# pastas/metran

Hardware: AMD Instinct MI355X
Metric: Kalman filter+smoother steps/sec (batched DFMs) (higher is better)
Workload: dtype f64

## Files before the change

include/metran_hip.h:

```cpp
#ifndef METRAN_HIP_H
#define METRAN_HIP_H

#include <stddef.h>
#include <stdint.h>

#ifdef __cplusplus
extern "C" {
#endif

#define MK_API __attribute__((visibility("default")))
#define MK_ABI_VERSION 7

typedef enum mk_status {
    MK_OK = 0,
    MK_ERR_INVALID = -1,
    MK_ERR_SHAPE = -2,
    MK_ERR_HIP = -3,
    MK_ERR_NO_DEVICE = -4,
    MK_ERR_ALLOC = -5
} mk_status;

#define MK_FLAG_NONPOSITIVE_F 1u
#define MK_FLAG_NOT_SPD 2u
#define MK_FLAG_RANK_DEFICIENT 4u
// ... 151 lines not shown
                           int64_t ndraws, int antithetic, int64_t T, int64_t ncomp, int raw, double *d_out);

MK_API int64_t mk_path_functional_count(void);
MK_API int mk_path_functionals(mk_context *ctx, const mk_problem *prob , int64_t ndraws,
                               int what , int time_major, const double *d_paths, int64_t W,
                               const int64_t *d_windows , const double *d_thresholds ,
                               double *d_functionals );
MK_API int64_t mk_ensemble_max_draws(void);
MK_API int mk_ensemble_summary(mk_context *ctx, int64_t S, int64_t cells, const double *d_values , int64_t nprobs,
                               const double *probs , double *d_summary );

typedef struct mk_weights_request {
    int64_t n_targets;
    int what;
    const int64_t *d_targets;
    double *d_weights;
    double *d_intercept;
} mk_weights_request;
MK_API int64_t mk_weights_work_stride(int64_t N, int64_t K);
MK_API int mk_observation_weights(mk_context *ctx, const mk_problem *prob, double *d_work, int time_major,
                                  const mk_weights_request *req, uint32_t *d_status);

MK_API int mk_smooth(mk_context *ctx, const mk_problem *prob, const mk_outputs *out);

MK_API int mk_filter_smooth(mk_context *ctx, const mk_problem *prob, const mk_outputs *out);

MK_API int mk_simulate(mk_context *ctx, int64_t B, int64_t RZ, int64_t T, int64_t N, int64_t n,
                       const double *d_Z, const double *d_means ,
                       const double *d_covs , double *d_sim_means ,
                       double *d_sim_vars );

MK_API int mk_decompose(mk_context *ctx, int64_t B, int64_t RZ, int64_t T, int64_t N, int64_t n,
                        const double *d_Z, const double *d_means ,
                        double *d_sdf , double *d_cdf );

MK_API int mk_sum(mk_context *ctx, int64_t count, const double *d_values, double *d_result );

MK_API int mk_comm_set_library(const char *path);
MK_API int mk_comm_unique_id(void *id128 );
MK_API int mk_comm_init_rank(mk_context *ctx, int nranks, int rank, const void *id128);
MK_API int mk_set_communicator(mk_context *ctx, void *nccl_comm);
MK_API int mk_comm_destroy(mk_context *ctx);
MK_API int mk_allreduce_sum(mk_context *ctx, double *d_buf, int64_t count);

MK_API int mk_standardize(mk_context *ctx, int64_t R, int64_t T, int64_t N, int time_major,
                          const double *d_in, double *d_out, double *d_mean, double *d_std);
// ... 29 lines not shown
```

metran_amd/_lib.py:

```python
import ctypes
import os
from ctypes import POINTER, Structure, c_char_p, c_double, c_float, c_int, c_int64, c_size_t, c_uint32, c_uint64, c_void_p

__all__ = ["MetranHipError", "lib", "library_path", "Problem", "Outputs", "ForecastRequest", "WeightsRequest", "check", "API"]

_HERE = os.path.dirname(os.path.abspath(__file__))
_LIBNAME = "libmetran_hip.so"


class MetranHipError(Exception):
    """Raised for every failure of the HIP library (the reference raises bare ``Exception``
    with a logged message, e.g. /root/reference/metran/kalmanfilter.py:733-745)."""


c_dp = POINTER(c_double)
c_i64p = POINTER(c_int64)
c_u32p = POINTER(c_uint32)


class Problem(Structure):

    _fields_ = [
        ("n_instances", c_int64),
        ("n_records", c_int64),
# ... 73 lines not shown
    "mk_sync": (c_int, [c_void_p]),
    "mk_observations_changed": (c_int, [c_void_p]),
    "mk_shape_supported": (c_int, [c_int64, c_int64]),
    "mk_shape_specialised": (c_int, [c_int64, c_int64]),
    "mk_generic_max_states": (c_int64, []),
    "mk_register_shape_module": (c_int, [c_char_p]),
    "mk_record_stride": (c_int64, [c_int64]),
    "mk_record_stride_sym": (c_int64, [c_int64]),
    "mk_tape_stride": (c_int64, [c_int64, c_int64]),
    "mk_tape_supported": (c_int, [c_int64, c_int64]),
    "mk_state_tape_stride": (c_int64, [c_int64, c_int64]),
    "mk_supported_shapes": (c_int, [c_i64p, c_int]),
    "mk_malloc": (c_int, [c_void_p, c_size_t, POINTER(c_void_p)]),
    "mk_free": (c_int, [c_void_p, c_void_p]),
    "mk_memcpy_h2d": (c_int, [c_void_p, c_void_p, c_void_p, c_size_t]),
    "mk_memcpy_d2h": (c_int, [c_void_p, c_void_p, c_void_p, c_size_t]),
    "mk_memset": (c_int, [c_void_p, c_void_p, c_int, c_size_t]),
    "mk_params_from_alpha": (c_int, [c_void_p, c_int64, c_int64, c_int64, c_int64, c_void_p, c_void_p, c_double,
                                     c_void_p, c_void_p]),
    "mk_filter": (c_int, [c_void_p, POINTER(Problem), POINTER(Outputs)]),
    "mk_loglik": (c_int, [c_void_p, POINTER(Problem), c_void_p]),
    "mk_smooth": (c_int, [c_void_p, POINTER(Problem), POINTER(Outputs)]),
    "mk_filter_smooth": (c_int, [c_void_p, POINTER(Problem), POINTER(Outputs)]),
    "mk_smooth_dense": (c_int, [c_void_p, c_int64, c_int64, c_int64, c_void_p, c_void_p, c_void_p, c_void_p, c_void_p, c_void_p,
                                c_void_p, c_void_p]),
    "mk_simulate": (c_int, [c_void_p, c_int64, c_int64, c_int64, c_int64, c_int64, c_void_p, c_void_p, c_void_p,
                            c_void_p, c_void_p]),
    "mk_decompose": (c_int, [c_void_p, c_int64, c_int64, c_int64, c_int64, c_int64, c_void_p, c_void_p, c_void_p,
                             c_void_p]),
    "mk_sum": (c_int, [c_void_p, c_int64, c_void_p, c_void_p]),
    "mk_comm_set_library": (c_int, [c_char_p]),
    "mk_comm_unique_id": (c_int, [c_void_p]),
    "mk_comm_init_rank": (c_int, [c_void_p, c_int, c_int, c_void_p]),
    "mk_set_communicator": (c_int, [c_void_p, c_void_p]),
    "mk_comm_destroy": (c_int, [c_void_p]),
    "mk_allreduce_sum": (c_int, [c_void_p, c_void_p, c_int64]),
    "mk_loglik_grad": (c_int, [c_void_p, POINTER(Problem), c_void_p, c_int, c_void_p, c_void_p, c_void_p, c_void_p, c_void_p]),
    "mk_loglik_grad_phases": (c_int, [c_void_p, POINTER(Problem), c_void_p, c_int, c_void_p, c_void_p, c_void_p, c_void_p, c_void_p,
                                      c_int]),
    "mk_adjoint_update_stride": (c_int64, [c_int64, c_int64]),
    "mk_set_adjoint_updates": (c_int, [c_void_p, c_void_p, c_int64]),
    "mk_lbfgs_direction": (c_int, [c_void_p, c_int64, c_int64, c_int64, c_void_p, c_void_p, c_void_p, c_void_p, c_void_p, c_void_p, c_void_p,
                                   c_void_p, c_void_p, c_double, c_void_p, c_void_p, c_void_p, c_void_p, c_void_p, POINTER(c_int)]),
    "mk_lbfgs_trial": (c_int, [c_void_p, c_int64, c_int64, c_void_p, c_void_p, c_void_p, c_void_p, c_void_p, c_void_p, c_void_p, c_void_p]),
    "mk_lbfgs_armijo": (c_int, [c_void_p, c_int64, c_int64, c_void_p, c_void_p, c_void_p, c_void_p, c_void_p, c_void_p, c_void_p, c_void_p,
                                c_void_p, c_void_p, c_int64, c_void_p, POINTER(c_int), POINTER(c_int)]),
# ... 82 lines not shown
```

metran_amd/csrc/mk_capi.hip:

```cpp
#include <hip/hip_runtime.h>

#include <cmath>
#include <cstdarg>
#include <cstdio>
#include <cstring>
#include <dlfcn.h>
#include <mutex>
#include <vector>
#include <new>

#include "draw_kernels.h"
#include "ensemble_kernels.h"
#include "forecast_kernels.h"
#include "innov_kernels.h"
#include "mk_generic.h"
#include "mk_internal.h"
#include "mk_lbfgs.h"
#include "weights_kernels.h"

struct mk_context {
    int device;
    hipStream_t stream;
    int timing;
    hipEvent_t ev[4];
    bool have_filter_time, have_smooth_time;
    std::vector<hipEvent_t> ev_pool;
    std::vector<std::pair<hipEvent_t, hipEvent_t>> ev_pending[2];
    int *tlist;
    long tlist_cap;
    const double *tlist_obs;
    long tlist_T, tlist_N, tlist_ostep;
    unsigned char *lr_take;
    long lr_cap;
    int *lr_any_dev;
    const double *lr_obs;
    long lr_R, lr_T, lr_N, lr_bs;
    int lr_any;
    int variant[MK_VARIANT_COUNT];
    double *gws;
    size_t gws_cap;
    int *lb_counters;
    double *adj_upd;
    size_t adj_upd_cap;
    double *cur_upd;
    void *comm;
    bool comm_owned;
};

static thread_local char g_err[512] = "";

static int fail(int code, const char *fmt, ...)
{
    va_list ap;
    va_start(ap, fmt);
    vsnprintf(g_err, sizeof(g_err), fmt, ap);
// ... 91 lines not shown
            hipError_t e = hipStreamSynchronize(ctx->stream);
            if (e != hipSuccess) return e;
            e = hipFree(ctx->gws);
            if (e != hipSuccess) return e;
        }
        ctx->gws = nullptr;
        ctx->gws_cap = 0;
        const hipError_t e = hipMalloc((void **)&ctx->gws, need * sizeof(double));
        if (e != hipSuccess) return e;
        ctx->gws_cap = need;
    }
    *ws = ctx->gws;
    return hipSuccess;
}
hipError_t dispatch_smoother(mk_context *ctx, int N, int K, const mk::SmootherArgs &a, hipStream_t s)
{
    const bool proj = a.sim_means || a.sim_vars || a.tape != 0;
    const bool force_generic = ctx->variant[MK_VARIANT_KERNEL_FAMILY] == 1;
    if (!force_generic) {
        if (const mk::ShapeOps *o = find_ops(N, K)) return o->smoother(a, s);
        if (!proj)
            if (const mk::ShapeOps *o = find_ops(N, K, true)) {
                mk::SmootherArgs b = a;
                b.obs = nullptr;
                return o->smoother(b, s);
            }
    }
    if (generic_shape(N, K)) {
        mk::GenericSmootherArgs g;
        g.a = a;
        g.N = N;
        g.K = K;
        g.Xp = g.Pp = nullptr;
        const hipError_t e = generic_workspace(ctx, a.B, N + K, &g.ws);
        if (e != hipSuccess) return e;
        return mk::launch_smoother_generic(g, s);
    }
    return hipErrorInvalidValue;
}
}

template <class Args>
static void fill_model(Args &a, const mk_problem *p)
{
    a.B = p->n_instances;
    a.R = p->n_records;
    a.T = p->T;
// ... 96 lines not shown
{
    if (!out) return fail(MK_ERR_INVALID, "null ctx out-pointer");
    *out = nullptr;
    int c = 0;
    if (hipGetDeviceCount(&c) != hipSuccess || c <= 0)
        return fail(MK_ERR_NO_DEVICE, "no HIP device visible (libmetran_hip needs an MI355X / gfx950)");
    if (device < 0 || device >= c) return fail(MK_ERR_INVALID, "device %d out of range [0,%d)", device, c);
    MK_HIP(hipSetDevice(device));
    hipDeviceProp_t prop;
    MK_HIP(hipGetDeviceProperties(&prop, device));
    if (strncmp(prop.gcnArchName, "gfx950", 6) != 0)
        return fail(MK_ERR_NO_DEVICE, "device %d is %s; this library is built for gfx950 only", device,
                    prop.gcnArchName);
    mk_context *ctx = new (std::nothrow) mk_context();
    if (!ctx) return fail(MK_ERR_ALLOC, "out of host memory");
    ctx->device = device;
    ctx->stream = nullptr;
    ctx->timing = 0;
    ctx->have_filter_time = ctx->have_smooth_time = false;
    ctx->tlist = nullptr;
    ctx->tlist_cap = 0;
    ctx->tlist_obs = nullptr;
    ctx->tlist_T = ctx->tlist_N = ctx->tlist_ostep = 0;
    ctx->lr_take = nullptr;
    ctx->lr_cap = 0;
    ctx->lr_any_dev = nullptr;
    ctx->lr_obs = nullptr;
    ctx->lr_R = ctx->lr_T = ctx->lr_N = ctx->lr_bs = 0;
    ctx->lr_any = 0;
    ctx->gws = nullptr;
    ctx->gws_cap = 0;
    ctx->lb_counters = nullptr;
    ctx->comm = nullptr;
    ctx->comm_owned = false;
    ctx->adj_upd = ctx->cur_upd = nullptr;
    ctx->adj_upd_cap = 0;
    for (int &v : ctx->variant) v = 0;
    for (auto &e : ctx->ev) {
        if (hipEventCreate(&e) != hipSuccess) {
            delete ctx;
            return fail(MK_ERR_HIP, "hipEventCreate failed");
        }
    }
    *out = ctx;
    return MK_OK;
}

// ... 122 lines not shown
        return fail(MK_ERR_INVALID, "mk_allreduce_sum: this context has no communicator -- call mk_comm_init_rank (every rank, with "
                                    "the id of mk_comm_unique_id) or mk_set_communicator first; there is no single-rank shortcut");
    if (!d_buf || count <= 0) return fail(MK_ERR_INVALID, "mk_allreduce_sum: bad argument");
    MK_HIP(hipSetDevice(ctx->device));
    const RcclApi *api = rccl_api();
    if (!api) return fail(MK_ERR_HIP, "mk_allreduce_sum: %s", g_rccl.why);
    MK_RCCL(api, api->AllReduce(d_buf, d_buf, (size_t)count, kNcclFloat64, kNcclSum, ctx->comm, ctx->stream));
    return MK_OK;
}

MK_API int mk_destroy(mk_context *ctx)
{
    if (!ctx) return MK_OK;
    (void)hipSetDevice(ctx->device);
    for (auto &e : ctx->ev) (void)hipEventDestroy(e);
    for (auto &e : ctx->ev_pool) (void)hipEventDestroy(e);
    for (auto &v : ctx->ev_pending)
        for (auto &pr : v) {
            (void)hipEventDestroy(pr.first);
            (void)hipEventDestroy(pr.second);
        }
    if (ctx->tlist) (void)hipFree(ctx->tlist);
    if (ctx->gws) (void)hipFree(ctx->gws);
    if (ctx->lr_take) (void)hipFree(ctx->lr_take);
    if (ctx->lr_any_dev) (void)hipFree(ctx->lr_any_dev);
    if (ctx->lb_counters) (void)hipFree(ctx->lb_counters);
    (void)mk_comm_destroy(ctx);
    delete ctx;
    return MK_OK;
}

MK_API int mk_set_stream(mk_context *ctx, void *s)
{
    MK_CTX(ctx);
    if (ctx->stream != (hipStream_t)s) ctx->tlist_obs = ctx->lr_obs = nullptr;
    ctx->stream = (hipStream_t)s;
    return MK_OK;
}

MK_API int mk_set_kernel_variant(mk_context *ctx, int which, int value)
{
    MK_CTX(ctx);
    if (which < 0 || which >= MK_VARIANT_COUNT) return fail(MK_ERR_INVALID, "mk_set_kernel_variant: unknown selector %d", which);
    if (value < 0 || value > ((which == MK_VARIANT_SINGLE_RECORD || which == MK_VARIANT_KERNEL_FAMILY || which == MK_VARIANT_TAPE_FILTER) ? 1 : 2))
        return fail(MK_ERR_INVALID, "mk_set_kernel_variant: value must be 0 or 1 (0, 1 or 2 for the smoother selectors and the wide filter)");
    ctx->variant[which] = value;
    return MK_OK;
// ... 257 lines not shown
    a.detfs = o->d_detfs;
    a.sigmacount = (long long *)o->d_sigmacount;
    a.F = o->d_F;
    a.Pf = o->d_Pf;
    a.Xp = o->d_Xp;
    a.Pp = o->d_Pp;
    a.status = o->d_status;
    if ((a.sym || a.tape) && (!specialised(p->N, p->K) || ctx->variant[MK_VARIANT_KERNEL_FAMILY] == 1))
        return fail(MK_ERR_SHAPE, "packed-symmetric records and the tape exist for specialised shapes only (N=%lld, K=%lld runs the size-generic "
                                  "kernels: mk_shape_specialised)", (long long)p->N, (long long)p->K);
    MK_HIP(timing_start(ctx, 0));
    {
        const hipError_t e = dispatch_filter((int)p->N, (int)p->K, a, ctx->stream, ctx->variant[MK_VARIANT_KERNEL_FAMILY] == 1);
        if (e == hipErrorNotSupported)
            return fail(MK_ERR_SHAPE, "a model of N=%lld series and K=%lld factors is not served on this device in this mode (the size-generic "
                                      "filter keeps the %lld x %lld covariance in LDS: %zu bytes)", (long long)p->N, (long long)p->K,
                        (long long)(p->N + p->K), (long long)(p->N + p->K), mk::generic_filter_lds_bytes((int)p->N, (int)p->K));
        MK_HIP(e);
    }
    MK_HIP(timing_stop(ctx, 0));
    return MK_OK;
}

static hipError_t full_records(mk_context *ctx, const mk_problem *p, const unsigned char **take)
{
    *take = nullptr;
    const long bs = p->obs_time_major ? 1 : p->T;
    if (!(ctx->lr_obs == p->d_obs && ctx->lr_R == p->n_records && ctx->lr_T == p->T && ctx->lr_N == p->N && ctx->lr_bs == bs)) {
        hipStreamCaptureStatus cap = hipStreamCaptureStatusNone;
        if (hipStreamIsCapturing(ctx->stream, &cap) != hipSuccess) (void)hipGetLastError();
        if (cap != hipStreamCaptureStatusNone) return hipSuccess;
        ctx->lr_obs = nullptr;
        if (ctx->lr_cap < p->n_records) {
            if (ctx->lr_take) {
                hipError_t e = hipStreamSynchronize(ctx->stream);
                if (e != hipSuccess) return e;
                (void)hipFree(ctx->lr_take);
                ctx->lr_take = nullptr;
                ctx->lr_cap = 0;
            }
            hipError_t e = hipMalloc((void **)&ctx->lr_take, (size_t)p->n_records);
            if (e != hipSuccess) return e;
            ctx->lr_cap = p->n_records;
        }
        if (!ctx->lr_any_dev) {
            hipError_t e = hipMalloc((void **)&ctx->lr_any_dev, sizeof(int));
            if (e != hipSuccess) return e;
        }
        hipError_t e = hipMemsetAsync(ctx->lr_any_dev, 0, sizeof(int), ctx->stream);
        if (e != hipSuccess) return e;
        e = mk::launch_full_records(p->n_records, p->T, (int)p->N, bs, p->obs_time_major ? p->n_records : 1, p->d_obs, ctx->lr_take,
                                    ctx->lr_any_dev, ctx->stream);
        if (e != hipSuccess) return e;
        e = hipMemcpyAsync(&ctx->lr_any, ctx->lr_any_dev, sizeof(int), hipMemcpyDeviceToHost, ctx->stream);
        if (e != hipSuccess) return e;
        e = hipStreamSynchronize(ctx->stream);
        if (e != hipSuccess) return e;
        ctx->lr_obs = p->d_obs;
        ctx->lr_R = p->n_records;
        ctx->lr_T = p->T;
        ctx->lr_N = p->N;
        ctx->lr_bs = bs;
    }
    if (ctx->lr_any) *take = ctx->lr_take;
    return hipSuccess;
}

static int do_smooth(mk_context *ctx, const mk_problem *p, const mk_outputs *o, bool clear_status)
{
    const int tape = tape_outputs(p, o);
    if (tape < 0) return tape;
    if (!o->d_F || (!o->d_Pf && !tape))
        return fail(MK_ERR_INVALID, "the smoother reads d_F and d_Pf (filtered moments); both must be non-NULL");
    if (tape == 1 && !(o->d_sim_means || o->d_sim_vars))
        return fail(MK_ERR_INVALID, "MK_OUT_TAPE: nothing to write, give d_sim_means / d_sim_vars");
    mk::SmootherArgs a;
    a.tape = tape;
    a.obsvar = tape ? p->d_obsvar : nullptr;
    a.variant = (ctx->variant[MK_VARIANT_SMOOTHER16] == 1 ? 1 : 0) | (ctx->variant[MK_VARIANT_WIDE_SMOOTHER] == 1 ? 2 : 0) |
                (ctx->variant[MK_VARIANT_WIDE_SMOOTHER] == 2 ? 4 : 0);
    a.rs = 0;
    a.sym = 0;
    a.state_means = a.state_vars = nullptr;
    const bool sym = (o->flags & MK_OUT_PACKED_SYM) != 0, var = (o->flags & MK_OUT_VAR_ONLY) != 0;
    if (tape) {
        a.rs = o->record_stride;
    } else if (o->record_stride) {
        const int64_t n = p->N + p->K;
        const int64_t want = sym ? mk::record_stride_sym((int)n) : mk::record_stride((int)n);
        if (o->record_stride != want)
            return fail(MK_ERR_INVALID, "record_stride must be %s(n) = %lld doubles", sym ? "mk_record_stride_sym" : "mk_record_stride",
                        (long long)want);
        const bool proj = o->d_sim_means || o->d_sim_vars;
        if (o->d_Pf != o->d_F + n) return fail(MK_ERR_INVALID, "record layout needs d_Pf = d_F + n");
        if (var) {
            if (!o->d_S || !o->d_Ps || proj)
                return fail(MK_ERR_INVALID, "MK_OUT_VAR_ONLY needs d_S [B,T,n] (means) and d_Ps [B,T,n] (variances), no projection outputs");
        } else {
            if ((o->d_S || o->d_Ps) && !(o->d_S && o->d_Ps == o->d_S + n))
                return fail(MK_ERR_INVALID, "record layout needs a smoothed record array d_S with d_Ps = d_S + n");
            if (!o->d_S && !proj)
                return fail(MK_ERR_INVALID, "nothing to write: give d_S/d_Ps records or d_sim_means/d_sim_vars");
        }
        if (proj && !p->d_loadings) return fail(MK_ERR_INVALID, "the projection outputs need d_loadings");
        a.rs = o->record_stride;
        a.sym = sym ? 1 : 0;
    } else if (o->d_sim_means || o->d_sim_vars || sym || var) {
        return fail(MK_ERR_INVALID, "d_sim_means / d_sim_vars, MK_OUT_PACKED_SYM and MK_OUT_VAR_ONLY need the record layout "
                                    "(record_stride = mk_record_stride[_sym](n))");
    }
    a.obs = nullptr;
    a.lr_take = nullptr;
    a.obs_bs = a.obs_ts = 0;
    if (p->d_obs && p->d_loadings && !p->d_obsvar && !tape && ctx->variant[MK_VARIANT_SMOOTHER16] != 2 &&
        (double)p->n_records * (double)p->T * (double)p->N * sizeof(double) < 4294967296.0) {
        const bool served = !sym && !var && o->record_stride && !(o->d_sim_means || o->d_sim_vars) && p->N + p->K <= 10 &&
                            ctx->variant[MK_VARIANT_SMOOTHER16] == 0 && ctx->variant[MK_VARIANT_KERNEL_FAMILY] == 0;
        if (served) MK_HIP(full_records(ctx, p, &a.lr_take));
        if (a.lr_take) {
            a.obs = p->d_obs;
            a.obs_bs = p->obs_time_major ? 1 : p->T;
            a.obs_ts = p->obs_time_major ? p->n_records : 1;
        }
    }
    a.R = p->n_records;
    a.loadings = p->d_loadings;
    fill_scaling(a, p);
    a.sim_means = o->d_sim_means;
    a.sim_vars = o->d_sim_vars;
    a.B = p->n_instances;
    a.T = p->T;
    fill_layout(a, (int)o->time_major, p->n_instances, p->T);
    a.phi = p->d_phi;
    a.q = p->d_q;
    a.F = o->d_F;
    a.Pf = o->d_Pf;
    if (tape == 2 && !p->d_loadings) return fail(MK_ERR_INVALID, "the state tape needs d_loadings");
    a.S = var ? nullptr : o->d_S;
    a.Ps = var ? nullptr : o->d_Ps;
    if (var) {
        a.state_means = o->d_S;
        a.state_vars = o->d_Ps;
    }
    a.status = o->d_status;
    MK_HIP(timing_start(ctx, 1));
    if ((sym || tape) && (!specialised(p->N, p->K) || ctx->variant[MK_VARIANT_KERNEL_FAMILY] == 1))
// ... 979 lines not shown
```

metran_amd/csrc/mk_ingest.hip:

```cpp
#include <hip/hip_runtime.h>

#include "mk_internal.h"

namespace mk {

__global__ void __launch_bounds__(256)
standardize_kernel(long R, long T, int N, long bs, long ts, const double *in, double *out, double *mean,
                   double *stdev)
{
    __shared__ double s_sum[256];
    __shared__ long s_cnt[256];
    __shared__ double s_mean[64], s_std[64];
    const long r = blockIdx.x;
    const int RP = 256 / N, tid = threadIdx.x;
    const int j = tid % N, row0 = tid / N;
    const bool active = row0 < RP;
    const double *src = in + r * bs * N;

    double acc = 0.0;
    long cnt = 0;
    if (active)
        for (long t = row0; t < T; t += RP) {
            const double y = src[t * ts * N + j];
            if (y == y) {
// ... 78 lines not shown
hipError_t launch_standardize(long R, long T, int N, int time_major, const double *in, double *out, double *mean,
                              double *stdev, hipStream_t s)
{
    const long bs = time_major ? 1 : T, ts = time_major ? R : 1;
    hipLaunchKernelGGL(standardize_kernel, dim3((unsigned)R), dim3(256), 0, s, R, T, N, bs, ts, in, out, mean, stdev);
    return hipGetLastError();
}

hipError_t launch_mask(long count, const double *obs, const unsigned char *mask, double *out, hipStream_t s)
{
    hipLaunchKernelGGL(mask_kernel, dim3((unsigned)((count + 255) / 256)), dim3(256), 0, s, count, obs, mask, out);
    return hipGetLastError();
}

hipError_t launch_pack(long RT, int N, const double *obs, double *observations, double *indices, long *count,
                       hipStream_t s)
{
    hipLaunchKernelGGL(pack_kernel, dim3((unsigned)((RT + 255) / 256)), dim3(256), 0, s, RT, N, obs, observations,
                       indices, count);
    return hipGetLastError();
}

__global__ void __launch_bounds__(256)
full_records_kernel(long T, int N, long obs_bs, long obs_ts, const double *obs, unsigned char *take, int *any)
{
    __shared__ unsigned s_cnt;
    if (threadIdx.x == 0) s_cnt = 0u;
    __syncthreads();
    const double *src = obs + (long)blockIdx.x * obs_bs * N;
    unsigned cnt = 0;
    for (long t = threadIdx.x; t < T; t += 256) {
        bool full = true;
        for (int j = 0; j < N; ++j) full = full && isfinite(src[t * obs_ts * N + j]);
        cnt += full ? 1u : 0u;
    }
    atomicAdd(&s_cnt, cnt);
    __syncthreads();
    if (threadIdx.x == 0) {
        const bool ok = 8ull * s_cnt >= 7ull * (unsigned long long)T;
        take[blockIdx.x] = ok ? 1 : 0;
        if (ok) atomicOr(any, 1);
    }
}

hipError_t launch_full_records(long R, long T, int N, long obs_bs, long obs_ts, const double *obs, unsigned char *take, int *any,
                               hipStream_t s)
{
    hipLaunchKernelGGL(full_records_kernel, dim3((unsigned)R), dim3(256), 0, s, T, N, obs_bs, obs_ts, obs, take, any);
    return hipGetLastError();
}

}
```

metran_amd/csrc/mk_internal.h:

```cpp
#pragma once
#include <hip/hip_runtime.h>

#include "metran_hip.h"

#ifndef MK_SHAPES
#define MK_SHAPES(X) \
    X(8, 2)          \
    X(5, 1)          \
    X(2, 1)          \
    X(3, 1)          \
    X(4, 1)          \
    X(6, 2)          \
    X(14, 3)         \
    X(32, 4)
#endif

namespace mk {

constexpr int wave_smoother_max_n = 51;

constexpr int tape_side_c(int K) { return K + 4; }
constexpr int tape_xs_c(int N, int K) { return N + tape_side_c(K); }
constexpr int tape_ss_c(int N, int K) { return tape_xs_c(N, K); }
constexpr int tape_so_c(int N, int K) { return N; }
// ... 23 lines not shown

#ifdef MK_TUNE
#define MK_TUNE_SKIP(args, bit) (((MK_TUNE) & (bit)) != 0)
#else
#define MK_TUNE_SKIP(args, bit) false
#endif

struct SmootherArgs {
    long B, T;
    long bs, ts;
    long rs;
    long sym;
    double *state_means, *state_vars;
    long R;
    const double *loadings, *scale, *offset;
    double *sim_means, *sim_vars;
    const double *phi, *q;
    const double *F, *Pf;
    double *S, *Ps;
    unsigned *status;
    long variant;
    long tape;
    const double *obsvar;
    const double *obs;
    long obs_bs, obs_ts;
    const unsigned char *lr_take;
};

struct AdjointArgs {
    long B, R, T, warmup;
    long bs, ts, rs;
    long obs_bs, obs_ts;
    const double *obs, *phi, *q, *loadings, *obsvar, *x0, *P0;
    const double *F;
    const long long *sigmacount;
    double *gphi, *gq;
    const double *upd;
    long us;
    double *loo_means, *loo_vars;
    const double *scale, *offset;
    double *dist_r, *dist_n;
};

enum class AdjointMode { Grad, Loo, Dist };

struct SparseArgs {
    long B, T, warmup;
    long ostep;
    const double *obs;
    const double *phi, *q, *loadings, *obsvar, *x0, *P0;
// ... 25 lines not shown
    hipError_t (*disturb)(const AdjointArgs &, hipStream_t);
};
const ShapeOps *shape_ops(int *count);
constexpr int module_abi()
{
    return (int)(sizeof(FilterArgs) * 1000 + sizeof(SmootherArgs) + sizeof(AdjointArgs) + sizeof(SparseArgs) + sizeof(ShapeOps));
}
hipError_t launch_alpha_grad(long B, long R, int N, int K, const double *alpha, const double *loadings, double dt,
                             const double *gphi, const double *gq, double *galpha, hipStream_t s);
int record_stride(int n);
int record_stride_sym(int n);
hipError_t launch_params(long B, long R, int N, int K, const double *alpha, const double *loadings, double dt,
                         double *phi, double *q, hipStream_t s);
hipError_t launch_simulate(long B, long RZ, long T, int N, int n, const double *Z, const double *means,
                           const double *covs, double *sm, double *sv, hipStream_t s);
hipError_t launch_decompose(long B, long RZ, long T, int N, int n, const double *Z, const double *means,
                            double *sdf, double *cdf, hipStream_t s);
hipError_t launch_sum(long count, const double *v, double *out, hipStream_t s);
hipError_t launch_standardize(long R, long T, int N, int time_major, const double *in, double *out, double *mean,
                              double *stdev, hipStream_t s);
hipError_t launch_mask(long count, const double *obs, const unsigned char *mask, double *out, hipStream_t s);
hipError_t launch_pack(long RT, int N, const double *obs, double *observations, double *indices, long *count,
                       hipStream_t s);
hipError_t launch_full_records(long R, long T, int N, long obs_bs, long obs_ts, const double *obs, unsigned char *take, int *any,
                               hipStream_t s);
hipError_t launch_fa_corr(long R, long T, int N, int time_major, const double *obs, double *corr, hipStream_t s);
hipError_t launch_fa_analyse(long B, int N, long maxfactors, const double *corr, double *eigval, long long *nfact,
                             long long *nfact_map, long long *nfact_map4, double *psi0, unsigned *status, hipStream_t s);
hipError_t launch_fa_minres(long B, long R, int N, int KMAX, const double *corr, const long long *nfact, const double *psi,
                            const long long *order, double *fval, double *grad, double *loadings, hipStream_t s);
hipError_t launch_fa_rotate(long B, int N, int KMAX, const long long *nfact, double *loadings, double gamma, int maxiter,
                            double tol, hipStream_t s);
hipError_t launch_fa_eigh(long B, int N, const double *sym, double *val, double *vec, hipStream_t s);

}
```

metran_amd/csrc/mk_kernels.hip:

```cpp
#include <cstdlib>
#include <cstring>

#include "mk_prims.h"

namespace mk {

template <int n, int G, bool SYM>
struct RecordIO;
#define MK_FILTER_WAVES(n, NK, OUT) ((((OUT) == 1 || (OUT) == 3) && (n) <= 10 && (NK) <= 16) ? 2 : 1)
template <int N>
constexpr int filter_gather_slot(int q) { return q < N - 1 ? q : N - 1; }
template <int N>
constexpr int filter_store_slot(int q) { return filter_gather_slot<N>(q) + 1; }

template <int N, int K, int G, int OUT, bool BOOK, bool SYM>
__global__ void __launch_bounds__(256) __attribute__((amdgpu_waves_per_eu(MK_FILTER_WAVES(N + K, N * K, OUT)))) filter_kernel(FilterArgs a)
{
    static_assert(G == 16, "a 16-lane group per model; wider models are filter_wave_kernel's");
    static_assert(OUT == 0 || OUT == 1 || OUT == 2 || OUT == 3, "the tape leaves the one-model-per-wavefront filter");
    static_assert(!SYM || OUT == 1 || OUT == 3, "packed-symmetric layout applies to record outputs");
    constexpr int n = N + K;
    static_assert(n <= G, "state dimension must fit the lane group");
    using Gp = Group<G>;
    constexpr int GPB = 256 / G;
// ... 885 lines not shown
    const long rec_id = inst % a.R;
    const int jr = lane < N ? lane : N - 1;
    double gam[K], pscale = 1.0, poffset = 0.0;
    double *pM = nullptr, *pV = nullptr;
    if constexpr (PROJ || LR) {
#pragma unroll
        for (int k = 0; k < K; ++k) gam[k] = a.loadings[(rec_id * N + jr) * K + k];
    }
    if constexpr (PROJ) {
        if (a.scale) pscale = a.scale[rec_id * N + jr];
        if (a.offset) poffset = a.offset[rec_id * N + jr];
        const long pidx = (inst * a.bs + (T - 1) * a.ts) * N + jr;
        pM = a.sim_means ? a.sim_means + pidx : nullptr;
        pV = a.sim_vars ? a.sim_vars + pidx : nullptr;
    }
    double *sM = nullptr, *sV = nullptr;
    if constexpr (VAR) {
        const long sidx = (inst * a.bs + (T - 1) * a.ts) * n + r;
        sM = a.state_means + sidx;
        sV = a.state_vars + sidx;
    }

    __shared__ double lds_gam[LR ? 256 * K : 1];
    __shared__ unsigned lds_ooff[LR ? 256 : 1];
    long otoff = 0, ostepb = 0;
    unsigned ooff = 0;
    int yhi = 0, wbase = 0;
    unsigned long long full_c = 0, full_n = 0;
    unsigned long long lr_models = 0;
    auto lane_now = [&]() __attribute__((always_inline)) {
        unsigned z = 0;
        asm volatile("" : "+v"(z));
        return (int)__builtin_amdgcn_mbcnt_hi(~0u, __builtin_amdgcn_mbcnt_lo(~0u, z));
    };
    if constexpr (LR) {
        ostepb = a.obs_ts * N * (long)sizeof(double);
        otoff = (T - 1) * ostepb;
        wbase = __builtin_amdgcn_readfirstlane((int)(threadIdx.x & ~63u));
#pragma unroll
        for (int k = 0; k < K; ++k) lds_gam[k * 256 + threadIdx.x] = gam[k];
        const unsigned mbase = (unsigned)(rec_id * a.obs_bs * N * (long)sizeof(double)) + 4u;
        lds_ooff[threadIdx.x] = mbase + (unsigned)jr * (unsigned)sizeof(double);
        lr_models = __ballot(a.lr_take[rec_id] != 0);
    }
    auto issue = [&](double &xnext) __attribute__((always_inline)) {
        recF -= rstep;
        RIO::load_issue(recF, rmap, prer);
        if constexpr (LR) {
            otoff -= ostepb;
            asm volatile("" : "+s"(otoff));
            yhi = *reinterpret_cast<const int *>(reinterpret_cast<const char *>(a.obs) + otoff + ooff);
        }
    };
    auto finish = [&](double &xv, double(&row)[n]) __attribute__((always_inline)) {
        if constexpr (LR) ooff = lds_ooff[wbase + lane_now()];
        RIO::load_finish(imgL, prer, rmap, gw, r, xv, row);
        if constexpr (LR) {
            unsigned long long m = __ballot((yhi & 0x7ff00000) != 0x7ff00000);
            m &= m >> 1;
            m &= m >> 2;
            m &= m >> 4;
            m &= m >> 8;
            m &= 0x0001000100010001ull;
            full_n = ((m << 16) - m) & lr_models;
        }
    };
    constexpr bool DEFER = (EPI == 0);
    auto store = [&](double xv, const double(&row)[n]) __attribute__((always_inline)) {
        if (recS) {
            RIO::put(imgS, gw, r, xv, row);
            if constexpr (!DEFER) {
                RIO::emit(imgS, recS, rmap);
                recS -= rstep;
            }
        }
        if constexpr (PROJ) {
            double mean, var;
            project<N, K, G>(xv, row, gam, pscale, poffset, lane, mean, var);
            if (lane < N && live) {
                if (pM) *pM = mean;
                if (pV) *pV = var;
            }
            if (pM) pM -= a.ts * N;
            if (pV) pV -= a.ts * N;
        }
        if constexpr (VAR) {
            double diag = 0.0;
            sfor<0, n>(MK_LAMBDA(c) { diag = (decltype(c)::value == lane) ? row[decltype(c)::value] : diag; });
            if (lane < n && live) {
                *sM = xv;
                *sV = diag;
            }
            sM -= a.ts * n;
            sV -= a.ts * n;
        }
    };
    typename RIO::chunk_t etmp[RIO::PER];

    double xs, Psn[n];
    RIO::load_issue(recF, rmap, prer);
    finish(xs, Psn);
    store(xs, Psn);
    double pivmin = 1.0;

    double Pfc[n], xfc = 0.0, xfn = 0.0;
    if (T >= 2) {
        issue(xfc);
        finish(xfc, Pfc);
        full_c = full_n;
        if (T >= 3) issue(xfn);
    }

    for (long t = T - 2; t >= 0; --t) {
        double A[n], z[n], D[n];
#pragma unroll
        for (int c = 0; c < n; ++c) {
            z[c] = Pfc[c] * phic[c];
            A[c] = fma(phi_r, z[c], qd[c]);
            D[c] = Psn[c] - A[c];
            if constexpr (DEFER) Psn[c] = Pfc[c];
        }
        double delta = xs - phi_r * xfc;
        if constexpr (G == 16) dpp_pin(delta);
        constexpr bool FACTOR_FWD = (G == 16) && Sweeps<n>::fused_factor && !SYM;
        if constexpr (FACTOR_FWD) {
#pragma unroll
            for (int c = 0; c < n; ++c) dpp_pin(D[c]);
        }

        if constexpr (DEFER)
            if (recS) RIO::gather_all(imgS, rmap, etmp);

// ... 54 lines not shown
        } else {
            sfor_down<0, n>(MK_LAMBDA(kc) {
                constexpr int k = decltype(kc)::value;
                Gp::template axpy_lane<k, 0, k, true, n>(z, A, z[k]);
            });
        }

        double acc0 = xfc, acc1 = 0.0;
        if constexpr (FUSED) {
            Sweeps<n>::mean(acc0, acc1, delta, z);
        } else {
            sfor<0, n>(MK_LAMBDA(cc) {
                constexpr int c = decltype(cc)::value;
                if constexpr (c % 2 == 0) Gp::template fmac<c>(acc0, delta, z[c]);
                else Gp::template fmac<c>(acc1, delta, z[c]);
            });
        }
        xs = acc0 + acc1;

        double V[n];
        if constexpr (G == 16) dpp_guard(D);
        if constexpr (LR) {
            const int ln = lane_now();
            if ((full_c >> ln) & 1ull) {
                double u[K], gl[K];
#pragma unroll
                for (int k = 0; k < K; ++k) gl[k] = lds_gam[k * 256 + wbase + ln];
                Sweeps<n>::lowrank(u, D, z);
                Sweeps<n>::lowrank_apply(Psn, u, gl);
            } else {
                Sweeps<n>::jd(V, D, z);
                Sweeps<n>::vjt(Psn, z, V);
            }
        } else if constexpr (FUSED) {
            Sweeps<n>::jd(V, D, z);
        } else {
#pragma unroll
            for (int c = 0; c < n; ++c) V[c] = 0.0;
            sfor<0, n>(MK_LAMBDA(kc) {
                constexpr int k = decltype(kc)::value;
                Gp::template axpy_lane<k, 0, n, false, n>(V, D, z[k]);
            });
        }
        if constexpr (!DEFER) {
#pragma unroll
            for (int c = 0; c < n; ++c) Psn[c] = Pfc[c];
        }
        if constexpr (LR) {
        } else if constexpr (FUSED) {
            Sweeps<n>::vjt(Psn, z, V);
        } else {
            sfor<0, n>(MK_LAMBDA(kc) {
                constexpr int k = decltype(kc)::value;
                Gp::template axpy_col<0, n, false, n>(Psn, z[k], V[k]);
            });
        }

        if constexpr (!DEFER) {
            if (t >= 1) {
                finish(xf_next, Pfc);
                if (t >= 2) issue(xfn);
            }
        }
        store(xs, Psn);
        xfc = xf_next;
        full_c = full_n;
    }
    if constexpr (DEFER)
        if (recS) RIO::emit(imgS, recS, rmap);
    if (a.status && live && lane == 0 && pivot_flags(pivmin)) atomicOr(a.status + inst, pivot_flags(pivmin));

}


template <int N, int K, bool SYM>
struct BlkLayout {
    static constexpr int n = N + K;
    using RIO = RecordIO<n, 16, SYM>;
    static constexpr int NBR = (n + 3) / 4;
    static constexpr int NBC = (n + 4) / 4;
    static constexpr int TR = 4 * NBR;
    static constexpr int TS = 20;
    static constexpr int IM = ((TR * TS - 8 + 31) / 32) * 32 + 8;
    static constexpr int DUMP = 4 * IM, ZERO = 4 * IM + 2;
    static constexpr int IMG = 4 * IM + 4;
    static constexpr int JR = 4 * NBR;
    static constexpr int JM = (n + 1) * JR;
    static constexpr int WAVE = 2 * IMG + 4 * JM;
    static_assert(n <= 15 && 4 * NBC <= TS, "the mean rides as column n of the tile");
// ... 1018 lines not shown
                if (a.sym) {
                    if (epi == 1) MK_LAUNCH_BLK(1, true);
                    else if (epi == 2) MK_LAUNCH_BLK(2, true);
                    else MK_LAUNCH_BLK(0, true);
                } else {
                    if (epi == 1) MK_LAUNCH_BLK(1, false);
                    else if (epi == 2) MK_LAUNCH_BLK(2, false);
                    else MK_LAUNCH_BLK(0, false);
                }
#undef MK_LAUNCH_BLK
                return hipGetLastError();
            }
        }
        if constexpr (G == 16 && Sweeps<n>::fused && K <= Sweeps<n>::lowrank_max_k) {
            static const bool keeps_occupancy = [] {
                int parent = 0, lowrank = 0;
                if (hipOccupancyMaxActiveBlocksPerMultiprocessor(&parent, smoother_record_kernel<N, K, G, 0, false, false>, 256, 0) != hipSuccess ||
                    hipOccupancyMaxActiveBlocksPerMultiprocessor(&lowrank, smoother_record_kernel<N, K, G, 0, false, true>, 256, 0) != hipSuccess) {
                    (void)hipGetLastError();
                    return false;
                }
                return lowrank > 0 && lowrank >= parent;
            }();
            if (a.rs > 0 && a.obs && epi == 0 && !a.sym && keeps_occupancy) {
                hipLaunchKernelGGL((smoother_record_kernel<N, K, G, 0, false, true>), dim3(grid), dim3(256), 0, s, a);
                return hipGetLastError();
            }
        }
        if (a.rs > 0) {
#define MK_LAUNCH_REC(E, S) hipLaunchKernelGGL((smoother_record_kernel<N, K, G, E, S>), dim3(grid), dim3(256), 0, s, a)
            if (a.sym) {
                if (epi == 1) MK_LAUNCH_REC(1, true);
                else if (epi == 2) MK_LAUNCH_REC(2, true);
                else MK_LAUNCH_REC(0, true);
            } else {
                if (epi == 1) MK_LAUNCH_REC(1, false);
                else if (epi == 2) MK_LAUNCH_REC(2, false);
                else MK_LAUNCH_REC(0, false);
            }
#undef MK_LAUNCH_REC
        } else
            hipLaunchKernelGGL((smoother_dense_kernel<n, G>), dim3(grid), dim3(256), 0, s, a);
    }
    return hipGetLastError();
}

int record_stride(int n) { return record_stride_c(n); }
// ... 142 lines not shown
```

metran_amd/engine.py:

```python
import ctypes
import logging

import numpy as np

from . import _lib
from ._lib import ForecastRequest, MetranHipError, Outputs, Problem, WeightsRequest, check

logger = logging.getLogger(__name__)

__all__ = ["BatchedKalman", "MetranHipError", "FLAG_NONPOSITIVE_F", "FLAG_NOT_SPD", "FLAG_RANK_DEFICIENT"]

FLAG_NONPOSITIVE_F = 1
FLAG_NOT_SPD = 2
FLAG_RANK_DEFICIENT = 4

_STATE_OUTPUTS = ("F", "Pf", "Xp", "Pp", "S", "Ps")


def _torch():
    import torch

    return torch


# ... 121 lines not shown
        return mean, std

    def mask_observations(self, mask):
        torch = _torch()
        if self.obs is None:
            raise MetranHipError("call set_observations first")
        base = self._obs_unmasked if getattr(self, "_obs_unmasked", None) is not None else self.obs
        if not isinstance(mask, torch.Tensor):
            mask = torch.from_numpy(np.ascontiguousarray(np.asarray(mask) != 0).view(np.uint8))
        mask = (mask != 0).to(device=self.device, dtype=torch.uint8)
        if mask.ndim == 2:
            mask = mask[None]
        if tuple(mask.shape) != (self.R, self.T, self.N):
            raise ValueError("Dimensions of mask %s do not equal dimensions of series %s"
                             % (tuple(mask.shape), (self.R, self.T, self.N)))
        mask = self._layout(mask)
        out = torch.empty_like(base)
        self._bind_stream()
        check(self._L.mk_mask_observations(self._ctx, int(base.numel()), self._p(base), self._p(mask), self._p(out)))
        self._obs_unmasked = base
        self.obs = out
        check(self._L.mk_observations_changed(self._ctx))
        return self

    def unmask_observations(self):
        if getattr(self, "_obs_unmasked", None) is not None:
            self.obs = self._obs_unmasked
            self._obs_unmasked = None
            check(self._L.mk_observations_changed(self._ctx))
        return self

    def pack_observations(self):
        torch = _torch()
        if self.obs is None:
            raise MetranHipError("call set_observations first")
        observations = torch.empty_like(self.obs)
        indices = torch.empty_like(self.obs)
        count = self._empty_bt(self.R, self.T, dtype=torch.int64)
        self._bind_stream()
        check(self._L.mk_pack_observations(self._ctx, self.R * self.T, 1, self.N, self._p(self.obs),
                                           self._p(observations), self._p(indices), self._p(count)))
        return observations, indices, count

    def _layout(self, t):
        if not self.time_major:
            return t.contiguous()
# ... 1005 lines not shown
```

Baseline: 1.412 billion.

## Precompute per-step full-observation bitmask instead of reading observations in smoother

The ingest kernel now writes a per-record bitmask marking which time steps have fully finite observations. The low-rank smoother reads one 32-bit word per 32 steps from constant address space instead of loading an observation word and reducing a wavefront ballot every step. This removes a strided global load and the ballot/shift reduction from the smoother's inner loop. It also drops the 4 GiB offset limit and adds a host API that exports the table, at the cost of a larger side buffer.

```diff
diff --git a/include/metran_hip.h b/include/metran_hip.h
--- a/include/metran_hip.h
+++ b/include/metran_hip.h
@@ -197,6 +197,8 @@
                                   const mk_weights_request *req, uint32_t *d_status);
 
 MK_API int mk_smooth(mk_context *ctx, const mk_problem *prob, const mk_outputs *out);
+MK_API int64_t mk_full_step_words(int64_t T);
+MK_API int mk_full_step_table(mk_context *ctx, const mk_problem *prob, uint32_t *h_words, int64_t capacity);
 
 MK_API int mk_filter_smooth(mk_context *ctx, const mk_problem *prob, const mk_outputs *out);
 
diff --git a/metran_amd/_lib.py b/metran_amd/_lib.py
--- a/metran_amd/_lib.py
+++ b/metran_amd/_lib.py
@@ -119,6 +119,8 @@
     "mk_loglik": (c_int, [c_void_p, POINTER(Problem), c_void_p]),
     "mk_smooth": (c_int, [c_void_p, POINTER(Problem), POINTER(Outputs)]),
     "mk_filter_smooth": (c_int, [c_void_p, POINTER(Problem), POINTER(Outputs)]),
+    "mk_full_step_words": (c_int64, [c_int64]),
+    "mk_full_step_table": (c_int, [c_void_p, POINTER(Problem), c_void_p, c_int64]),
     "mk_smooth_dense": (c_int, [c_void_p, c_int64, c_int64, c_int64, c_void_p, c_void_p, c_void_p, c_void_p, c_void_p, c_void_p,
                                 c_void_p, c_void_p]),
     "mk_simulate": (c_int, [c_void_p, c_int64, c_int64, c_int64, c_int64, c_int64, c_void_p, c_void_p, c_void_p,
diff --git a/metran_amd/csrc/mk_capi.hip b/metran_amd/csrc/mk_capi.hip
--- a/metran_amd/csrc/mk_capi.hip
+++ b/metran_amd/csrc/mk_capi.hip
@@ -30,7 +30,7 @@
     long tlist_cap;
     const double *tlist_obs;
     long tlist_T, tlist_N, tlist_ostep;
-    unsigned char *lr_take;
+    unsigned *lr_bits;
     long lr_cap;
     int *lr_any_dev;
     const double *lr_obs;
@@ -168,7 +168,7 @@
         if (!proj)
             if (const mk::ShapeOps *o = find_ops(N, K, true)) {
                 mk::SmootherArgs b = a;
-                b.obs = nullptr;
+                b.lr_bits = nullptr;
                 return o->smoother(b, s);
             }
     }
@@ -311,7 +311,7 @@
     ctx->tlist_cap = 0;
     ctx->tlist_obs = nullptr;
     ctx->tlist_T = ctx->tlist_N = ctx->tlist_ostep = 0;
-    ctx->lr_take = nullptr;
+    ctx->lr_bits = nullptr;
     ctx->lr_cap = 0;
     ctx->lr_any_dev = nullptr;
     ctx->lr_obs = nullptr;
@@ -480,7 +480,7 @@
         }
     if (ctx->tlist) (void)hipFree(ctx->tlist);
     if (ctx->gws) (void)hipFree(ctx->gws);
-    if (ctx->lr_take) (void)hipFree(ctx->lr_take);
+    if (ctx->lr_bits) (void)hipFree(ctx->lr_bits);
     if (ctx->lr_any_dev) (void)hipFree(ctx->lr_any_dev);
     if (ctx->lb_counters) (void)hipFree(ctx->lb_counters);
     (void)mk_comm_destroy(ctx);
@@ -784,26 +784,27 @@
     return MK_OK;
 }
 
-static hipError_t full_records(mk_context *ctx, const mk_problem *p, const unsigned char **take)
-{
-    *take = nullptr;
+static hipError_t full_records(mk_context *ctx, const mk_problem *p, const unsigned **bits)
+{
+    *bits = nullptr;
     const long bs = p->obs_time_major ? 1 : p->T;
     if (!(ctx->lr_obs == p->d_obs && ctx->lr_R == p->n_records && ctx->lr_T == p->T && ctx->lr_N == p->N && ctx->lr_bs == bs)) {
         hipStreamCaptureStatus cap = hipStreamCaptureStatusNone;
         if (hipStreamIsCapturing(ctx->stream, &cap) != hipSuccess) (void)hipGetLastError();
         if (cap != hipStreamCaptureStatusNone) return hipSuccess;
         ctx->lr_obs = nullptr;
-        if (ctx->lr_cap < p->n_records) {
-            if (ctx->lr_take) {
+        const long words = p->n_records * mk::full_step_words(p->T);
+        if (ctx->lr_cap < words) {
+            if (ctx->lr_bits) {
                 hipError_t e = hipStreamSynchronize(ctx->stream);
                 if (e != hipSuccess) return e;
-                (void)hipFree(ctx->lr_take);
-                ctx->lr_take = nullptr;
+                (void)hipFree(ctx->lr_bits);
+                ctx->lr_bits = nullptr;
                 ctx->lr_cap = 0;
             }
-            hipError_t e = hipMalloc((void **)&ctx->lr_take, (size_t)p->n_records);
+            hipError_t e = hipMalloc((void **)&ctx->lr_bits, (size_t)words * sizeof(unsigned));
             if (e != hipSuccess) return e;
-            ctx->lr_cap = p->n_records;
+            ctx->lr_cap = words;
         }
         if (!ctx->lr_any_dev) {
             hipError_t e = hipMalloc((void **)&ctx->lr_any_dev, sizeof(int));
@@ -811,7 +812,7 @@
         }
         hipError_t e = hipMemsetAsync(ctx->lr_any_dev, 0, sizeof(int), ctx->stream);
         if (e != hipSuccess) return e;
-        e = mk::launch_full_records(p->n_records, p->T, (int)p->N, bs, p->obs_time_major ? p->n_records : 1, p->d_obs, ctx->lr_take,
+        e = mk::launch_full_records(p->n_records, p->T, (int)p->N, bs, p->obs_time_major ? p->n_records : 1, p->d_obs, ctx->lr_bits,
                                     ctx->lr_any_dev, ctx->stream);
         if (e != hipSuccess) return e;
         e = hipMemcpyAsync(&ctx->lr_any, ctx->lr_any_dev, sizeof(int), hipMemcpyDeviceToHost, ctx->stream);
@@ -824,8 +825,27 @@
         ctx->lr_N = p->N;
         ctx->lr_bs = bs;
     }
-    if (ctx->lr_any) *take = ctx->lr_take;
+    if (ctx->lr_any) *bits = ctx->lr_bits;
     return hipSuccess;
+}
+
+MK_API int64_t mk_full_step_words(int64_t T) { return T > 0 ? (int64_t)mk::full_step_words(T) : 0; }
+
+MK_API int mk_full_step_table(mk_context *ctx, const mk_problem *p, uint32_t *h_words, int64_t capacity)
+{
+    MK_CTX(ctx);
+    if (!p || p->n_records <= 0 || p->T <= 0 || p->N <= 0 || !p->d_obs || !h_words)
+        return fail(MK_ERR_INVALID, "mk_full_step_table: need n_records, T, N >= 1, prob->d_obs and h_words");
+    const int64_t words = p->n_records * (int64_t)mk::full_step_words(p->T);
+    if (capacity < words)
+        return fail(MK_ERR_INVALID, "mk_full_step_table: h_words holds %lld words, the table has n_records * mk_full_step_words(T) = %lld",
+                    (long long)capacity, (long long)words);
+    const unsigned *bits = nullptr;
+    MK_HIP(full_records(ctx, p, &bits));
+    if (!ctx->lr_obs) return fail(MK_ERR_INVALID, "mk_full_step_table: not while the stream is being captured");
+    MK_HIP(hipMemcpyAsync(h_words, ctx->lr_bits, (size_t)words * sizeof(uint32_t), hipMemcpyDeviceToHost, ctx->stream));
+    MK_HIP(hipStreamSynchronize(ctx->stream));
+    return MK_OK;
 }
 
 static int do_smooth(mk_context *ctx, const mk_problem *p, const mk_outputs *o, bool clear_status)
@@ -871,19 +891,13 @@
         return fail(MK_ERR_INVALID, "d_sim_means / d_sim_vars, MK_OUT_PACKED_SYM and MK_OUT_VAR_ONLY need the record layout "
                                     "(record_stride = mk_record_stride[_sym](n))");
     }
-    a.obs = nullptr;
-    a.lr_take = nullptr;
-    a.obs_bs = a.obs_ts = 0;
-    if (p->d_obs && p->d_loadings && !p->d_obsvar && !tape && ctx->variant[MK_VARIANT_SMOOTHER16] != 2 &&
-        (double)p->n_records * (double)p->T * (double)p->N * sizeof(double) < 4294967296.0) {
+    a.lr_bits = nullptr;
+    a.lr_words = a.lr_unused[0] = a.lr_unused[1] = 0;
+    if (p->d_obs && p->d_loadings && !p->d_obsvar && !tape && ctx->variant[MK_VARIANT_SMOOTHER16] != 2) {
         const bool served = !sym && !var && o->record_stride && !(o->d_sim_means || o->d_sim_vars) && p->N + p->K <= 10 &&
                             ctx->variant[MK_VARIANT_SMOOTHER16] == 0 && ctx->variant[MK_VARIANT_KERNEL_FAMILY] == 0;
-        if (served) MK_HIP(full_records(ctx, p, &a.lr_take));
-        if (a.lr_take) {
-            a.obs = p->d_obs;
-            a.obs_bs = p->obs_time_major ? 1 : p->T;
-            a.obs_ts = p->obs_time_major ? p->n_records : 1;
-        }
+        if (served) MK_HIP(full_records(ctx, p, &a.lr_bits));
+        if (a.lr_bits) a.lr_words = mk::full_step_words(p->T);
     }
     a.R = p->n_records;
     a.loadings = p->d_loadings;
diff --git a/metran_amd/csrc/mk_ingest.hip b/metran_amd/csrc/mk_ingest.hip
--- a/metran_amd/csrc/mk_ingest.hip
+++ b/metran_amd/csrc/mk_ingest.hip
@@ -124,31 +124,38 @@
 }
 
 __global__ void __launch_bounds__(256)
-full_records_kernel(long T, int N, long obs_bs, long obs_ts, const double *obs, unsigned char *take, int *any)
+full_records_kernel(long T, int N, long obs_bs, long obs_ts, const double *obs, unsigned *bits, int *any)
 {
     __shared__ unsigned s_cnt;
     if (threadIdx.x == 0) s_cnt = 0u;
     __syncthreads();
     const double *src = obs + (long)blockIdx.x * obs_bs * N;
-    unsigned cnt = 0;
-    for (long t = threadIdx.x; t < T; t += 256) {
+    auto full_at = [&](long t) {
         bool full = true;
         for (int j = 0; j < N; ++j) full = full && isfinite(src[t * obs_ts * N + j]);
-        cnt += full ? 1u : 0u;
-    }
+        return full;
+    };
+    unsigned cnt = 0;
+    for (long t = threadIdx.x; t < T; t += 256) cnt += full_at(t) ? 1u : 0u;
     atomicAdd(&s_cnt, cnt);
     __syncthreads();
-    if (threadIdx.x == 0) {
-        const bool ok = 8ull * s_cnt >= 7ull * (unsigned long long)T;
-        take[blockIdx.x] = ok ? 1 : 0;
-        if (ok) atomicOr(any, 1);
+    const bool ok = 8ull * s_cnt >= 7ull * (unsigned long long)T;
+    if (threadIdx.x == 0 && ok) atomicOr(any, 1);
+    const long W = full_step_words(T);
+    unsigned *row = bits + (long)blockIdx.x * W;
+    const int lane = threadIdx.x & 63;
+    for (long t0 = threadIdx.x - lane; t0 < T; t0 += 256) {
+        const long t = t0 + lane;
+        const unsigned long long m = __ballot(ok && t < T && full_at(t));
+        const long w = (t0 >> 5) + lane;
+        if (lane < 2 && w < W) row[w] = (unsigned)(m >> (32 * lane));
     }
 }
 
-hipError_t launch_full_records(long R, long T, int N, long obs_bs, long obs_ts, const double *obs, unsigned char *take, int *any,
+hipError_t launch_full_records(long R, long T, int N, long obs_bs, long obs_ts, const double *obs, unsigned *bits, int *any,
                                hipStream_t s)
 {
-    hipLaunchKernelGGL(full_records_kernel, dim3((unsigned)R), dim3(256), 0, s, T, N, obs_bs, obs_ts, obs, take, any);
+    hipLaunchKernelGGL(full_records_kernel, dim3((unsigned)R), dim3(256), 0, s, T, N, obs_bs, obs_ts, obs, bits, any);
     return hipGetLastError();
 }
 
diff --git a/metran_amd/csrc/mk_internal.h b/metran_amd/csrc/mk_internal.h
--- a/metran_amd/csrc/mk_internal.h
+++ b/metran_amd/csrc/mk_internal.h
@@ -69,10 +69,11 @@
     long variant;
     long tape;
     const double *obsvar;
-    const double *obs;
-    long obs_bs, obs_ts;
-    const unsigned char *lr_take;
+    const unsigned *lr_bits;
+    long lr_words;
+    long lr_unused[2];
 };
+constexpr long full_step_words(long T) { return (T + 31) / 32; }
 
 struct AdjointArgs {
     long B, R, T, warmup;
@@ -144,7 +145,7 @@
 hipError_t launch_mask(long count, const double *obs, const unsigned char *mask, double *out, hipStream_t s);
 hipError_t launch_pack(long RT, int N, const double *obs, double *observations, double *indices, long *count,
                        hipStream_t s);
-hipError_t launch_full_records(long R, long T, int N, long obs_bs, long obs_ts, const double *obs, unsigned char *take, int *any,
+hipError_t launch_full_records(long R, long T, int N, long obs_bs, long obs_ts, const double *obs, unsigned *bits, int *any,
                                hipStream_t s);
 hipError_t launch_fa_corr(long R, long T, int N, int time_major, const double *obs, double *corr, hipStream_t s);
 hipError_t launch_fa_analyse(long B, int N, long maxfactors, const double *corr, double *eigval, long long *nfact,
diff --git a/metran_amd/csrc/mk_kernels.hip b/metran_amd/csrc/mk_kernels.hip
--- a/metran_amd/csrc/mk_kernels.hip
+++ b/metran_amd/csrc/mk_kernels.hip
@@ -931,48 +931,42 @@
     }
 
     __shared__ double lds_gam[LR ? 256 * K : 1];
-    __shared__ unsigned lds_ooff[LR ? 256 : 1];
-    long otoff = 0, ostepb = 0;
-    unsigned ooff = 0;
-    int yhi = 0, wbase = 0;
-    unsigned long long full_c = 0, full_n = 0;
-    unsigned long long lr_models = 0;
+    int wbase = 0;
+    typedef const unsigned __attribute__((address_space(4))) *bits_ptr;
+    bits_ptr bitrow[4] = {nullptr, nullptr, nullptr, nullptr};
+    unsigned bw_c[4] = {0u, 0u, 0u, 0u};
     auto lane_now = [&]() __attribute__((always_inline)) {
         unsigned z = 0;
         asm volatile("" : "+v"(z));
         return (int)__builtin_amdgcn_mbcnt_hi(~0u, __builtin_amdgcn_mbcnt_lo(~0u, z));
     };
     if constexpr (LR) {
-        ostepb = a.obs_ts * N * (long)sizeof(double);
-        otoff = (T - 1) * ostepb;
         wbase = __builtin_amdgcn_readfirstlane((int)(threadIdx.x & ~63u));
 #pragma unroll
         for (int k = 0; k < K; ++k) lds_gam[k * 256 + threadIdx.x] = gam[k];
-        const unsigned mbase = (unsigned)(rec_id * a.obs_bs * N * (long)sizeof(double)) + 4u;
-        lds_ooff[threadIdx.x] = mbase + (unsigned)jr * (unsigned)sizeof(double);
-        lr_models = __ballot(a.lr_take[rec_id] != 0);
-    }
+        const long woff = rec_id * a.lr_words;
+        const long wi = (T - 2) >> 5;
+#pragma unroll
+        for (int g = 0; g < 4; ++g) {
+            const unsigned lo = (unsigned)__builtin_amdgcn_readlane((int)(unsigned)woff, 16 * g);
+            const unsigned hi = (unsigned)__builtin_amdgcn_readlane((int)(unsigned)((unsigned long)woff >> 32), 16 * g);
+            bitrow[g] = (bits_ptr)(unsigned long)a.lr_bits + (long)(((unsigned long)hi << 32) | lo);
+            if (T >= 2) bw_c[g] = bitrow[g][wi];
+        }
+    }
+    auto full_mask = [&](long t) __attribute__((always_inline)) {
+        const unsigned b = (unsigned)t & 31u;
+        const unsigned m0 = 0u - ((bw_c[0] >> b) & 1u), m1 = 0u - ((bw_c[1] >> b) & 1u);
+        const unsigned m2 = 0u - ((bw_c[2] >> b) & 1u), m3 = 0u - ((bw_c[3] >> b) & 1u);
+        const unsigned lo = (m0 & 0x0000ffffu) | (m1 & 0xffff0000u), hi = (m2 & 0x0000ffffu) | (m3 & 0xffff0000u);
+        return ((unsigned long long)hi << 32) | lo;
+    };
     auto issue = [&](double &xnext) __attribute__((always_inline)) {
         recF -= rstep;
         RIO::load_issue(recF, rmap, prer);
-        if constexpr (LR) {
-            otoff -= ostepb;
-            asm volatile("" : "+s"(otoff));
-            yhi = *reinterpret_cast<const int *>(reinterpret_cast<const char *>(a.obs) + otoff + ooff);
-        }
     };
     auto finish = [&](double &xv, double(&row)[n]) __attribute__((always_inline)) {
-        if constexpr (LR) ooff = lds_ooff[wbase + lane_now()];
         RIO::load_finish(imgL, prer, rmap, gw, r, xv, row);
-        if constexpr (LR) {
-            unsigned long long m = __ballot((yhi & 0x7ff00000) != 0x7ff00000);
-            m &= m >> 1;
-            m &= m >> 2;
-            m &= m >> 4;
-            m &= m >> 8;
-            m &= 0x0001000100010001ull;
-            full_n = ((m << 16) - m) & lr_models;
-        }
     };
     constexpr bool DEFER = (EPI == 0);
     auto store = [&](double xv, const double(&row)[n]) __attribute__((always_inline)) {
@@ -1016,7 +1010,6 @@
     if (T >= 2) {
         issue(xfc);
         finish(xfc, Pfc);
-        full_c = full_n;
         if (T >= 3) issue(xfn);
     }
 
@@ -1117,7 +1110,7 @@
         if constexpr (G == 16) dpp_guard(D);
         if constexpr (LR) {
             const int ln = lane_now();
-            if ((full_c >> ln) & 1ull) {
+            if ((full_mask(t) >> ln) & 1ull) {
                 double u[K], gl[K];
 #pragma unroll
                 for (int k = 0; k < K; ++k) gl[k] = lds_gam[k * 256 + wbase + ln];
@@ -1159,7 +1152,12 @@
         }
         store(xs, Psn);
         xfc = xf_next;
-        full_c = full_n;
+        if constexpr (LR) {
+            if ((t & 31) == 0 && t > 0) {
+#pragma unroll
+                for (int g = 0; g < 4; ++g) bw_c[g] = bitrow[g][(t >> 5) - 1];
+            }
+        }
     }
     if constexpr (DEFER)
         if (recS) RIO::emit(imgS, recS, rmap);
@@ -2224,7 +2222,7 @@
                 }
                 return lowrank > 0 && lowrank >= parent;
             }();
-            if (a.rs > 0 && a.obs && epi == 0 && !a.sym && keeps_occupancy) {
+            if (a.rs > 0 && a.lr_bits && epi == 0 && !a.sym && keeps_occupancy) {
                 hipLaunchKernelGGL((smoother_record_kernel<N, K, G, 0, false, true>), dim3(grid), dim3(256), 0, s, a);
                 return hipGetLastError();
             }
diff --git a/metran_amd/engine.py b/metran_amd/engine.py
--- a/metran_amd/engine.py
+++ b/metran_amd/engine.py
@@ -167,6 +167,17 @@
         self.obs = out
         check(self._L.mk_observations_changed(self._ctx))
         return self
+
+    def full_step_table(self):
+        if self.obs is None:
+            raise MetranHipError("call set_observations first")
+        W = int(self._L.mk_full_step_words(self.T))
+        out = np.empty((self.R, W), dtype=np.uint32)
+        prob = Problem(self.R, self.R, self.T, self.N, 1, 0, self._p(self.obs), None, None, None, None, None, None,
+                       1 if self.time_major else 0, None, None)
+        self._bind_stream()
+        check(self._L.mk_full_step_table(self._ctx, ctypes.byref(prob), ctypes.c_void_p(out.ctypes.data), out.size))
+        return out
 
     def unmask_observations(self):
         if getattr(self, "_obs_unmasked", None) is not None:
```

Result: no change. 1.419 billion, median of 6 (+0.5%).
